# 10XGenomics/thermite

Measured on AMD Instinct MI355X. Metric: aligned reads/sec (91 bp), higher is better.
Workload: dtype i32

## Files before the change

thermite_amd/csrc/kernels_compact.hip:

```cpp
#include <hip/hip_runtime.h>

#include <algorithm>
#include <cstddef>
#include <cstdlib>

#include "launch.h"

namespace thm {
namespace dev {

constexpr uint32_t COMPACT_HEAVY_N = 8, COMPACT_CHUNK = 4;

struct CandRegs {
  uint32_t lo, hi;
};
static_assert(sizeof(Cand) == 112 && sizeof(thm_aln) == 112, "compact_emit permutes the dwords of these layouts");
static_assert(offsetof(Cand, ops_off) == 48 && offsetof(Cand, tx_ops_off) == 56 && offsetof(Cand, score) == 64 &&
                  offsetof(Cand, ops_len) == 80 && offsetof(Cand, tx_ops_len) == 84 && offsetof(Cand, strand) == 108 &&
                  offsetof(thm_aln, ops_off) == 24 && offsetof(thm_aln, tx_ops_off) == 56 && offsetof(thm_aln, xlen) == 80 &&
                  offsetof(thm_aln, ops_len) == 84 && offsetof(thm_aln, tx_ops_len) == 104 && offsetof(thm_aln, strand) == 108,
              "compact_emit permutes the dwords of these layouts");

__device__ __forceinline__ CandRegs cand_load(const Cand* c, int sub) {
  const uint32_t* w = reinterpret_cast<const uint32_t*>(c);
  CandRegs r;
  r.lo = w[sub];
  r.hi = sub < 12 ? w[16 + sub] : 0u;
  return r;
}

__device__ __forceinline__ uint32_t compact_emit(const CompactParams& p, const CandRegs c, uint64_t ai, uint64_t o, uint32_t xlen, bool primary, int sub) {
  const uint64_t ops_off = (uint64_t)__shfl(c.lo, 12, 16) | ((uint64_t)__shfl(c.lo, 13, 16) << 32);
  const uint64_t tx_ops_off = (uint64_t)__shfl(c.lo, 14, 16) | ((uint64_t)__shfl(c.lo, 15, 16) << 32);
  const uint32_t ops_len = __shfl(c.hi, 4, 16), tx_ops_len = __shfl(c.hi, 5, 16), flags = __shfl(c.hi, 11, 16);
  if (ai >= p.alns_cap || o + ops_len + tx_ops_len > p.ops_cap) return ops_len + tx_ops_len;
  auto copy_ops = [&](const uint8_t* src, uint8_t* dst, uint32_t len) {
    #pragma unroll 1
    for (uint32_t b0 = 0; b0 < len; b0 += 64) {
      uint8_t v[4];
      #pragma unroll
      for (int k = 0; k < 4; k++) {
        const uint32_t b = b0 + (uint32_t)sub + 16u * (uint32_t)k;
        v[k] = (b < len) ? src[b] : (uint8_t)0;
      }
      #pragma unroll
      for (int k = 0; k < 4; k++) {
        const uint32_t b = b0 + (uint32_t)sub + 16u * (uint32_t)k;
        if (b < len) dst[b] = v[k];
      }
    }
  };
  copy_ops(p.cand_ops + ops_off, p.ops + o, ops_len);
  const uint64_t go = o, to = o + ops_len;
  copy_ops(p.cand_ops + tx_ops_off, p.ops + to, tx_ops_len);
  const int src_lo = (int)((0x00BA987600543210ull >> (4 * sub)) & 15u);
  const int src_hi = (int)((0x0000B59876403210ull >> (4 * sub)) & 15u);
  uint32_t w0 = __shfl(c.lo, src_lo, 16), w1 = __shfl(c.hi, src_hi, 16);
  const uint64_t txo = ((flags >> 8) & 0xFFu) == THM_ALN_EXONIC ? to : 0ull;
  if (sub == 6) w0 = (uint32_t)go;
  if (sub == 7) w0 = (uint32_t)(go >> 32);
  if (sub == 14) w0 = (uint32_t)txo;
  if (sub == 15) w0 = (uint32_t)(txo >> 32);
  if (sub == 4) w1 = xlen;
  if (sub == 11) w1 = (flags & 0xFFu) | ((primary ? 1u : 0u) << 8) | (((flags >> 8) & 0xFFu) << 16);
  uint32_t* out = reinterpret_cast<uint32_t*>(p.alns + ai);
  out[sub] = w0;
  if (sub < 12) out[16 + sub] = w1;
  return ops_len + tx_ops_len;
}

__device__ __forceinline__ bool compact_faulted(const CompactParams& p) { return p.fault[0] != 0 || (p.fault[1] & FAULT_OPS_POOL) != 0; }

template <int K>
__global__ __launch_bounds__(256) void compact_kernel(CompactParams p) {
  const int sub = (int)(threadIdx.x & 15u);
  if (compact_faulted(p)) return;
  const uint64_t n_groups = (uint64_t)gridDim.x * 16, g = ((uint64_t)blockIdx.x * 256 + threadIdx.x) >> 4;
  for (uint64_t rb = g; rb < p.n_reads; rb += (uint64_t)K * n_groups) {
    uint32_t n[K], xlen[K], l0[K];
    uint64_t cand0[K], a0[K], o[K];
    #pragma unroll
    for (int k = 0; k < K; k++) {
      const uint64_t r = rb + (uint64_t)k * n_groups;
      n[k] = r < p.n_reads ? p.read_n_alns[r] : 0u;
    }
    #pragma unroll
    for (int k = 0; k < K; k++) {
      const uint64_t r = rb + (uint64_t)k * n_groups;
      if (n[k] > COMPACT_HEAVY_N) {
        if (sub == 0) {
          const unsigned long long h = atomicAdd(&p.heavy_cnt[0], 1ull);
          if (h < p.heavy_cap) p.heavy_list[h] = r;
        }
        n[k] = 0;
      }
      if (n[k]) {
        cand0[k] = p.read_cand_off[r];
        a0[k] = p.read_aln_off[r];
        o[k] = p.read_ops_off[r];
        xlen[k] = (uint32_t)(p.read_offsets[r + 1] - p.read_offsets[r]);
      }
    }
    #pragma unroll
    for (int k = 0; k < K; k++)
      if (n[k]) l0[k] = p.order[2 * cand0[k]];
    CandRegs cd[K];
    #pragma unroll
    for (int k = 0; k < K; k++)
      if (n[k]) cd[k] = cand_load(p.cands + cand0[k] + l0[k], sub);
    #pragma unroll
    for (int k = 0; k < K; k++) {
      if (!n[k]) continue;
      uint64_t ok = o[k] + compact_emit(p, cd[k], a0[k], o[k], xlen[k], true, sub);
      const uint32_t* la = p.order + 2 * cand0[k];
      for (uint32_t t = 1; t < n[k]; t++)
        ok += compact_emit(p, cand_load(p.cands + cand0[k] + la[t], sub), a0[k] + t, ok, xlen[k], false, sub);
    }
  }
}

__global__ __launch_bounds__(256) void compact_heavy_scan_kernel(CompactParams p) {
  __shared__ uint32_t wave_sum[4];
  __shared__ unsigned long long desc_base;
  if (compact_faulted(p)) return;
  const uint64_t H = min((unsigned long long)p.heavy_cap, p.heavy_cnt[0]);
  const int tid = (int)threadIdx.x, lane = tid & 63, wv = tid >> 6;
  for (uint64_t h = blockIdx.x; h < H; h += gridDim.x) {
    const uint64_t r = p.heavy_list[h];
    const uint32_t n = p.read_n_alns[r];
    const uint64_t cand0 = p.read_cand_off[r], a0 = p.read_aln_off[r];
    const Cand* cands = p.cands + cand0;
    const uint32_t* la = p.order + 2 * cand0;
    uint32_t carry = 0;
    for (uint32_t tile = 0; tile < n; tile += 256) {
      const uint32_t t = tile + (uint32_t)tid;
      uint32_t len = 0;
      if (t < n) {
        const Cand* cd = &cands[la[t]];
        len = cd->ops_len + cd->tx_ops_len;
      }
      uint32_t inc = len;
      #pragma unroll
      for (int o = 1; o < 64; o <<= 1) {
        const uint32_t v = __shfl_up(inc, o);
        if (lane >= o) inc += v;
      }
      if (lane == 63) wave_sum[wv] = inc;
      __syncthreads();
      uint32_t before = carry, total = 0;
      #pragma unroll
      for (int k = 0; k < 4; k++) {
        if (k < wv) before += wave_sum[k];
        total += wave_sum[k];
      }
      if (t < n && a0 + t < p.alns_cap) p.rel[a0 + t] = before + inc - len;
      carry += total;
      __syncthreads();
    }
    const uint32_t nd = (n + COMPACT_CHUNK - 1) / COMPACT_CHUNK;
    if (tid == 0) desc_base = atomicAdd(&p.heavy_cnt[1], (unsigned long long)nd);
    __syncthreads();
    const unsigned long long base = desc_base;
    for (uint32_t k = (uint32_t)tid; k < nd; k += 256)
      if (base + k < p.heavy_cap) p.heavy_desc[base + k] = (r << 24) | (uint64_t)k;
    __syncthreads();
  }
}

__global__ __launch_bounds__(256) void compact_heavy_copy_kernel(CompactParams p) {
  const int sub = (int)(threadIdx.x & 15u);
  if (compact_faulted(p)) return;
  const uint64_t D = min((unsigned long long)p.heavy_cap, p.heavy_cnt[1]);
  const uint64_t n_groups = (uint64_t)gridDim.x * 16;
  for (uint64_t d = ((uint64_t)blockIdx.x * 256 + threadIdx.x) >> 4; d < D; d += n_groups) {
    const uint64_t desc = p.heavy_desc[d], r = desc >> 24;
    const uint32_t t0 = (uint32_t)(desc & 0xFFFFFFu) * COMPACT_CHUNK, n = p.read_n_alns[r];
    const uint64_t cand0 = p.read_cand_off[r], a0 = p.read_aln_off[r], o0 = p.read_ops_off[r];
    const Cand* cands = p.cands + cand0;
    const uint32_t* la = p.order + 2 * cand0;
    const uint32_t xlen = (uint32_t)(p.read_offsets[r + 1] - p.read_offsets[r]);
    for (uint32_t t = t0; t < n && t < t0 + COMPACT_CHUNK; t++) {
      if (a0 + t >= p.alns_cap) break;
      (void)compact_emit(p, cand_load(&cands[la[t]], sub), a0 + t, o0 + p.rel[a0 + t], xlen, t == 0, sub);
    }
  }
}

}

int compact_k() {
  static const int v = [] {
    const char* e = getenv("THM_COMPACT_K");
    const int v = e ? atoi(e) : 2;
    return v == 1 || v == 2 || v == 4 ? v : 2;
  }();
  return v;
}

hipError_t launch_compact(const CompactParams& p, hipStream_t s) {
  static const unsigned n_cu = [] {
    int dev = 0, cu = 256;
    if (hipGetDevice(&dev) == hipSuccess) (void)hipDeviceGetAttribute(&cu, hipDeviceAttributeMultiprocessorCount, dev);
    return (unsigned)cu;
  }();
  const unsigned blocks = (unsigned)std::min<uint64_t>((p.n_reads + 15) / 16, (uint64_t)n_cu * 8);
  if (blocks == 0) return hipSuccess;
  const int k_reads = compact_k();
  if (k_reads == 1)
    hipLaunchKernelGGL(dev::compact_kernel<1>, dim3(blocks), dim3(256), 0, s, p);
  else if (k_reads == 2)
    hipLaunchKernelGGL(dev::compact_kernel<2>, dim3(blocks), dim3(256), 0, s, p);
  else
    hipLaunchKernelGGL(dev::compact_kernel<4>, dim3(blocks), dim3(256), 0, s, p);
  hipLaunchKernelGGL(dev::compact_heavy_scan_kernel, dim3(n_cu), dim3(256), 0, s, p);
  hipLaunchKernelGGL(dev::compact_heavy_copy_kernel, dim3(n_cu * 4), dim3(256), 0, s, p);
  return hipGetLastError();
}

}
```

Measured before the change: 93.87 million.

## Restructure compact kernel: per-alignment LDS work slots and dword-aligned ops copy

The compact kernel now gives each thread one read. Those threads stage per-alignment copy descriptors into shared-memory slots, and 16-lane groups then process alignments (not reads) in batches of K, issuing all loads before any stores. The byte-at-a-time ops copy is replaced by a dword copy aligned to the destination, with funnel shifts for source misalignment and single-byte head and tail handling, and a waitcnt separates the load and store phases. This aims to cut memory instructions and to balance work across lanes when reads carry different numbers of alignments. In exchange it adds shared-memory pressure, block-level syncs, serial descriptor generation per thread, and possible unaligned 32-bit source reads.

```diff
diff --git a/thermite_amd/csrc/compact_copy.h b/thermite_amd/csrc/compact_copy.h
--- /dev/null
+++ b/thermite_amd/csrc/compact_copy.h
@@ -0,0 +1,85 @@
+#ifndef THERMITE_COMPACT_COPY_H
+#define THERMITE_COMPACT_COPY_H
+#include <cstdint>
+
+#if defined(__HIPCC__)
+#define CCOPY_HD __host__ __device__ inline
+#else
+#define CCOPY_HD inline
+#endif
+
+namespace thm {
+namespace ccopy {
+
+constexpr int LANES = 16;
+constexpr int DWORDS_PER_LANE = 4;
+constexpr uint32_t TRIP_DWORDS = (uint32_t)(LANES * DWORDS_PER_LANE);
+constexpr uint32_t NO_BYTE = 0xFFFFFFFFu;
+constexpr int TAIL_LANE0 = 8;
+
+CCOPY_HD uint32_t head_bytes(uint64_t dst, uint32_t len) {
+  const uint32_t h = (uint32_t)(0 - dst) & 3u;
+  return h < len ? h : len;
+}
+CCOPY_HD uint32_t body_dwords(uint64_t dst, uint32_t len) { return (len - head_bytes(dst, len)) >> 2; }
+CCOPY_HD uint32_t tail_bytes(uint64_t dst, uint32_t len) { return (len - head_bytes(dst, len)) & 3u; }
+CCOPY_HD uint32_t trips(uint64_t dst, uint32_t len) {
+  const uint32_t nd = body_dwords(dst, len);
+  return nd ? (nd + TRIP_DWORDS - 1) / TRIP_DWORDS : (len ? 1u : 0u);
+}
+CCOPY_HD uint32_t lane_dword(int lane, int m, uint32_t trip) { return trip * TRIP_DWORDS + (uint32_t)m * LANES + (uint32_t)lane; }
+CCOPY_HD uint32_t edge_byte(int lane, uint64_t dst, uint32_t len) {
+  const uint32_t head = head_bytes(dst, len), tail = tail_bytes(dst, len);
+  if ((uint32_t)lane < head) return (uint32_t)lane;
+  if (lane >= TAIL_LANE0 && (uint32_t)(lane - TAIL_LANE0) < tail) return len - tail + (uint32_t)(lane - TAIL_LANE0);
+  return NO_BYTE;
+}
+CCOPY_HD uint32_t funnel(uint32_t lo, uint32_t hi, uint32_t shift) { return shift ? (lo >> (8 * shift)) | (hi << (32 - 8 * shift)) : lo; }
+
+struct LaneRegs {
+  uint32_t lo[DWORDS_PER_LANE], hi[DWORDS_PER_LANE];
+  uint32_t edge;
+};
+
+template <class M>
+CCOPY_HD void lane_load(const M& mem, uint64_t src, uint64_t dst, uint32_t len, uint32_t trip, int lane, LaneRegs& r) {
+  const uint32_t head = head_bytes(dst, len), nd = body_dwords(dst, len);
+#if defined(__HIPCC__)
+  #pragma unroll
+#endif
+  for (int m = 0; m < DWORDS_PER_LANE; m++) {
+    const uint32_t j = lane_dword(lane, m, trip);
+    r.lo[m] = r.hi[m] = 0u;
+    if (j < nd) {
+      const uint64_t s = src + head + 4ull * j;
+      r.lo[m] = mem.ld32(s & ~3ull);
+      if (s & 3u) r.hi[m] = mem.ld32((s & ~3ull) + 4);
+    }
+  }
+  r.edge = 0u;
+  if (trip == 0) {
+    const uint32_t e = edge_byte(lane, dst, len);
+    if (e != NO_BYTE) r.edge = mem.ld8(src + e);
+  }
+}
+
+template <class M>
+CCOPY_HD void lane_store(M& mem, uint64_t src, uint64_t dst, uint32_t len, uint32_t trip, int lane, const LaneRegs& r) {
+  const uint32_t head = head_bytes(dst, len), nd = body_dwords(dst, len);
+  const uint32_t shift = (uint32_t)(src + head) & 3u;
+#if defined(__HIPCC__)
+  #pragma unroll
+#endif
+  for (int m = 0; m < DWORDS_PER_LANE; m++) {
+    const uint32_t j = lane_dword(lane, m, trip);
+    if (j < nd) mem.st32(dst + head + 4ull * j, funnel(r.lo[m], r.hi[m], shift));
+  }
+  if (trip == 0) {
+    const uint32_t e = edge_byte(lane, dst, len);
+    if (e != NO_BYTE) mem.st8(dst + e, (uint8_t)r.edge);
+  }
+}
+
+}
+}
+#endif
diff --git a/thermite_amd/csrc/kernels_compact.hip b/thermite_amd/csrc/kernels_compact.hip
--- a/thermite_amd/csrc/kernels_compact.hip
+++ b/thermite_amd/csrc/kernels_compact.hip
@@ -4,6 +4,7 @@
 #include <cstddef>
 #include <cstdlib>
 
+#include "compact_copy.h"
 #include "launch.h"
 
 namespace thm {
@@ -14,12 +15,12 @@
 struct CandRegs {
   uint32_t lo, hi;
 };
-static_assert(sizeof(Cand) == 112 && sizeof(thm_aln) == 112, "compact_emit permutes the dwords of these layouts");
+static_assert(sizeof(Cand) == 112 && sizeof(thm_aln) == 112, "emit_record permutes the dwords of these layouts");
 static_assert(offsetof(Cand, ops_off) == 48 && offsetof(Cand, tx_ops_off) == 56 && offsetof(Cand, score) == 64 &&
                   offsetof(Cand, ops_len) == 80 && offsetof(Cand, tx_ops_len) == 84 && offsetof(Cand, strand) == 108 &&
                   offsetof(thm_aln, ops_off) == 24 && offsetof(thm_aln, tx_ops_off) == 56 && offsetof(thm_aln, xlen) == 80 &&
                   offsetof(thm_aln, ops_len) == 84 && offsetof(thm_aln, tx_ops_len) == 104 && offsetof(thm_aln, strand) == 108,
-              "compact_emit permutes the dwords of these layouts");
+              "emit_record permutes the dwords of these layouts");
 
 __device__ __forceinline__ CandRegs cand_load(const Cand* c, int sub) {
   const uint32_t* w = reinterpret_cast<const uint32_t*>(c);
@@ -29,93 +30,139 @@
   return r;
 }
 
-__device__ __forceinline__ uint32_t compact_emit(const CompactParams& p, const CandRegs c, uint64_t ai, uint64_t o, uint32_t xlen, bool primary, int sub) {
-  const uint64_t ops_off = (uint64_t)__shfl(c.lo, 12, 16) | ((uint64_t)__shfl(c.lo, 13, 16) << 32);
-  const uint64_t tx_ops_off = (uint64_t)__shfl(c.lo, 14, 16) | ((uint64_t)__shfl(c.lo, 15, 16) << 32);
-  const uint32_t ops_len = __shfl(c.hi, 4, 16), tx_ops_len = __shfl(c.hi, 5, 16), flags = __shfl(c.hi, 11, 16);
-  if (ai >= p.alns_cap || o + ops_len + tx_ops_len > p.ops_cap) return ops_len + tx_ops_len;
-  auto copy_ops = [&](const uint8_t* src, uint8_t* dst, uint32_t len) {
+struct OpsMem {
+  const uint8_t* src;
+  uint8_t* dst;
+  __device__ __forceinline__ uint32_t ld32(uint64_t o) const { return *reinterpret_cast<const uint32_t*>(src + o); }
+  __device__ __forceinline__ uint32_t ld8(uint64_t o) const { return src[o]; }
+  __device__ __forceinline__ void st32(uint64_t o, uint32_t v) { *reinterpret_cast<uint32_t*>(dst + o) = v; }
+  __device__ __forceinline__ void st8(uint64_t o, uint8_t v) { dst[o] = v; }
+};
+
+struct AlnCopy {
+  CandRegs c;
+  ccopy::LaneRegs gx, tx;
+  uint64_t gx_src, tx_src, o;
+  uint32_t gx_len, tx_len;
+
+  __device__ __forceinline__ void load(const CompactParams& p, const Cand* cand, uint64_t gx_src_, uint64_t tx_src_, uint32_t gx_len_, uint32_t tx_len_,
+                                       uint64_t o_, int sub) {
+    gx_src = gx_src_, tx_src = tx_src_, gx_len = gx_len_, tx_len = tx_len_, o = o_;
+    const OpsMem mem{p.cand_ops, p.ops};
+    c = cand_load(cand, sub);
+    ccopy::lane_load(mem, gx_src, o, gx_len, 0, sub, gx);
+    ccopy::lane_load(mem, tx_src, o + gx_len, tx_len, 0, sub, tx);
+  }
+
+  static __device__ __forceinline__ void loads_done() { __builtin_amdgcn_s_waitcnt(0x0F70); }
+
+  __device__ __forceinline__ void store(const CompactParams& p, uint64_t ai, uint32_t xlen, bool primary, int sub) {
+    OpsMem mem{p.cand_ops, p.ops};
+    const uint64_t go = o, to = o + gx_len;
+    ccopy::lane_store(mem, gx_src, go, gx_len, 0, sub, gx);
+    ccopy::lane_store(mem, tx_src, to, tx_len, 0, sub, tx);
     #pragma unroll 1
-    for (uint32_t b0 = 0; b0 < len; b0 += 64) {
-      uint8_t v[4];
-      #pragma unroll
-      for (int k = 0; k < 4; k++) {
-        const uint32_t b = b0 + (uint32_t)sub + 16u * (uint32_t)k;
-        v[k] = (b < len) ? src[b] : (uint8_t)0;
-      }
-      #pragma unroll
-      for (int k = 0; k < 4; k++) {
-        const uint32_t b = b0 + (uint32_t)sub + 16u * (uint32_t)k;
-        if (b < len) dst[b] = v[k];
-      }
-    }
-  };
-  copy_ops(p.cand_ops + ops_off, p.ops + o, ops_len);
-  const uint64_t go = o, to = o + ops_len;
-  copy_ops(p.cand_ops + tx_ops_off, p.ops + to, tx_ops_len);
-  const int src_lo = (int)((0x00BA987600543210ull >> (4 * sub)) & 15u);
-  const int src_hi = (int)((0x0000B59876403210ull >> (4 * sub)) & 15u);
-  uint32_t w0 = __shfl(c.lo, src_lo, 16), w1 = __shfl(c.hi, src_hi, 16);
-  const uint64_t txo = ((flags >> 8) & 0xFFu) == THM_ALN_EXONIC ? to : 0ull;
-  if (sub == 6) w0 = (uint32_t)go;
-  if (sub == 7) w0 = (uint32_t)(go >> 32);
-  if (sub == 14) w0 = (uint32_t)txo;
-  if (sub == 15) w0 = (uint32_t)(txo >> 32);
-  if (sub == 4) w1 = xlen;
-  if (sub == 11) w1 = (flags & 0xFFu) | ((primary ? 1u : 0u) << 8) | (((flags >> 8) & 0xFFu) << 16);
-  uint32_t* out = reinterpret_cast<uint32_t*>(p.alns + ai);
-  out[sub] = w0;
-  if (sub < 12) out[16 + sub] = w1;
-  return ops_len + tx_ops_len;
-}
+    for (uint32_t trip = 1; trip < ccopy::trips(go, gx_len); trip++) {
+      ccopy::lane_load(mem, gx_src, go, gx_len, trip, sub, gx);
+      loads_done();
+      ccopy::lane_store(mem, gx_src, go, gx_len, trip, sub, gx);
+    }
+    #pragma unroll 1
+    for (uint32_t trip = 1; trip < ccopy::trips(to, tx_len); trip++) {
+      ccopy::lane_load(mem, tx_src, to, tx_len, trip, sub, tx);
+      loads_done();
+      ccopy::lane_store(mem, tx_src, to, tx_len, trip, sub, tx);
+    }
+    const uint32_t flags = __shfl(c.hi, 11, 16);
+    const int src_lo = (int)((0x00BA987600543210ull >> (4 * sub)) & 15u);
+    const int src_hi = (int)((0x0000B59876403210ull >> (4 * sub)) & 15u);
+    uint32_t w0 = __shfl(c.lo, src_lo, 16), w1 = __shfl(c.hi, src_hi, 16);
+    const uint64_t txo = ((flags >> 8) & 0xFFu) == THM_ALN_EXONIC ? to : 0ull;
+    if (sub == 6) w0 = (uint32_t)go;
+    if (sub == 7) w0 = (uint32_t)(go >> 32);
+    if (sub == 14) w0 = (uint32_t)txo;
+    if (sub == 15) w0 = (uint32_t)(txo >> 32);
+    if (sub == 4) w1 = xlen;
+    if (sub == 11) w1 = (flags & 0xFFu) | ((primary ? 1u : 0u) << 8) | (((flags >> 8) & 0xFFu) << 16);
+    uint32_t* out = reinterpret_cast<uint32_t*>(p.alns + ai);
+    out[sub] = w0;
+    if (sub < 12) out[16 + sub] = w1;
+  }
+};
 
 __device__ __forceinline__ bool compact_faulted(const CompactParams& p) { return p.fault[0] != 0 || (p.fault[1] & FAULT_OPS_POOL) != 0; }
 
+constexpr uint32_t COMPACT_TILE = 256, COMPACT_SLOTS = 512;
+constexpr uint64_t NO_CAND = ~0ull;
+
 template <int K>
-__global__ __launch_bounds__(256) void compact_kernel(CompactParams p) {
-  const int sub = (int)(threadIdx.x & 15u);
+__global__ __launch_bounds__(COMPACT_TILE) void compact_kernel(CompactParams p) {
+  __shared__ uint64_t s_cand[COMPACT_SLOTS], s_gx[COMPACT_SLOTS], s_tx[COMPACT_SLOTS], s_o[COMPACT_SLOTS];
+  __shared__ uint32_t s_gx_len[COMPACT_SLOTS], s_tx_len[COMPACT_SLOTS], s_xlen[COMPACT_SLOTS];
+  __shared__ uint8_t s_primary[COMPACT_SLOTS];
   if (compact_faulted(p)) return;
-  const uint64_t n_groups = (uint64_t)gridDim.x * 16, g = ((uint64_t)blockIdx.x * 256 + threadIdx.x) >> 4;
-  for (uint64_t rb = g; rb < p.n_reads; rb += (uint64_t)K * n_groups) {
-    uint32_t n[K], xlen[K], l0[K];
-    uint64_t cand0[K], a0[K], o[K];
-    #pragma unroll
-    for (int k = 0; k < K; k++) {
-      const uint64_t r = rb + (uint64_t)k * n_groups;
-      n[k] = r < p.n_reads ? p.read_n_alns[r] : 0u;
-    }
-    #pragma unroll
-    for (int k = 0; k < K; k++) {
-      const uint64_t r = rb + (uint64_t)k * n_groups;
-      if (n[k] > COMPACT_HEAVY_N) {
-        if (sub == 0) {
-          const unsigned long long h = atomicAdd(&p.heavy_cnt[0], 1ull);
-          if (h < p.heavy_cap) p.heavy_list[h] = r;
-        }
-        n[k] = 0;
-      }
-      if (n[k]) {
-        cand0[k] = p.read_cand_off[r];
-        a0[k] = p.read_aln_off[r];
-        o[k] = p.read_ops_off[r];
-        xlen[k] = (uint32_t)(p.read_offsets[r + 1] - p.read_offsets[r]);
-      }
-    }
-    #pragma unroll
-    for (int k = 0; k < K; k++)
-      if (n[k]) l0[k] = p.order[2 * cand0[k]];
-    CandRegs cd[K];
-    #pragma unroll
-    for (int k = 0; k < K; k++)
-      if (n[k]) cd[k] = cand_load(p.cands + cand0[k] + l0[k], sub);
-    #pragma unroll
-    for (int k = 0; k < K; k++) {
-      if (!n[k]) continue;
-      uint64_t ok = o[k] + compact_emit(p, cd[k], a0[k], o[k], xlen[k], true, sub);
-      const uint32_t* la = p.order + 2 * cand0[k];
-      for (uint32_t t = 1; t < n[k]; t++)
-        ok += compact_emit(p, cand_load(p.cands + cand0[k] + la[t], sub), a0[k] + t, ok, xlen[k], false, sub);
-    }
+  const uint32_t tid = threadIdx.x;
+  const int sub = (int)(tid & 15u);
+  const uint32_t grp = tid >> 4;
+  const uint64_t r0 = (uint64_t)blockIdx.x * COMPACT_TILE, r = r0 + tid;
+  const uint64_t r_end = min((unsigned long long)(r0 + COMPACT_TILE), (unsigned long long)p.n_reads);
+  const uint64_t aln_base = p.read_aln_off[r0], n_slots = p.read_aln_off[r_end] - aln_base;
+  uint32_t n = 0, xlen = 0;
+  uint64_t cand0 = 0, a0 = 0, o = 0;
+  if (r < p.n_reads) {
+    n = p.read_n_alns[r];
+    cand0 = p.read_cand_off[r];
+    a0 = p.read_aln_off[r];
+    o = p.read_ops_off[r];
+    xlen = (uint32_t)(p.read_offsets[r + 1] - p.read_offsets[r]);
+  }
+  if (n > COMPACT_HEAVY_N) {
+    const unsigned long long h = atomicAdd(&p.heavy_cnt[0], 1ull);
+    if (h < p.heavy_cap) p.heavy_list[h] = r;
+    n = 0;
+  }
+  uint32_t t = 0;
+  for (uint64_t c0 = 0; c0 < n_slots; c0 += COMPACT_SLOTS) {
+    const uint32_t cnt = (uint32_t)min((unsigned long long)COMPACT_SLOTS, (unsigned long long)(n_slots - c0));
+    for (uint32_t i = tid; i < cnt; i += COMPACT_TILE) s_cand[i] = NO_CAND;
+    __syncthreads();
+    while (t < n && a0 + t - aln_base < c0 + COMPACT_SLOTS) {
+      const uint32_t slot = (uint32_t)(a0 + t - aln_base - c0);
+      const uint64_t ci = cand0 + p.order[2 * cand0 + t];
+      const Cand* cd = p.cands + ci;
+      const uint64_t gx_src = cd->ops_off, tx_src = cd->tx_ops_off;
+      const uint32_t gx_len = cd->ops_len, tx_len = cd->tx_ops_len;
+      if (a0 + t < p.alns_cap && o + gx_len + tx_len <= p.ops_cap) {
+        s_cand[slot] = ci;
+        s_gx[slot] = gx_src;
+        s_tx[slot] = tx_src;
+        s_o[slot] = o;
+        s_gx_len[slot] = gx_len;
+        s_tx_len[slot] = tx_len;
+        s_xlen[slot] = xlen;
+        s_primary[slot] = t == 0;
+      }
+      o += gx_len + tx_len;
+      t++;
+    }
+    __syncthreads();
+    for (uint32_t b = 0; b < cnt; b += 16 * K) {
+      AlnCopy ac[K];
+      bool live[K];
+      #pragma unroll
+      for (int k = 0; k < K; k++) {
+        const uint32_t d = b + grp + 16u * (uint32_t)k;
+        live[k] = d < cnt && s_cand[d] != NO_CAND;
+        if (live[k]) ac[k].load(p, p.cands + s_cand[d], s_gx[d], s_tx[d], s_gx_len[d], s_tx_len[d], s_o[d], sub);
+      }
+      AlnCopy::loads_done();
+      #pragma unroll
+      for (int k = 0; k < K; k++) {
+        const uint32_t d = b + grp + 16u * (uint32_t)k;
+        if (live[k]) ac[k].store(p, aln_base + c0 + d, s_xlen[d], s_primary[d] != 0, sub);
+      }
+    }
+    __syncthreads();
   }
 }
 
@@ -181,7 +228,14 @@
     const uint32_t xlen = (uint32_t)(p.read_offsets[r + 1] - p.read_offsets[r]);
     for (uint32_t t = t0; t < n && t < t0 + COMPACT_CHUNK; t++) {
       if (a0 + t >= p.alns_cap) break;
-      (void)compact_emit(p, cand_load(&cands[la[t]], sub), a0 + t, o0 + p.rel[a0 + t], xlen, t == 0, sub);
+      const Cand* cd = &cands[la[t]];
+      const uint32_t gx_len = cd->ops_len, tx_len = cd->tx_ops_len;
+      const uint64_t o = o0 + p.rel[a0 + t];
+      if (o + gx_len + tx_len > p.ops_cap) continue;
+      AlnCopy ac;
+      ac.load(p, cd, cd->ops_off, cd->tx_ops_off, gx_len, tx_len, o, sub);
+      AlnCopy::loads_done();
+      ac.store(p, a0 + t, xlen, t == 0, sub);
     }
   }
 }
@@ -203,15 +257,15 @@
     if (hipGetDevice(&dev) == hipSuccess) (void)hipDeviceGetAttribute(&cu, hipDeviceAttributeMultiprocessorCount, dev);
     return (unsigned)cu;
   }();
-  const unsigned blocks = (unsigned)std::min<uint64_t>((p.n_reads + 15) / 16, (uint64_t)n_cu * 8);
+  const unsigned blocks = (unsigned)((p.n_reads + dev::COMPACT_TILE - 1) / dev::COMPACT_TILE);
   if (blocks == 0) return hipSuccess;
-  const int k_reads = compact_k();
-  if (k_reads == 1)
-    hipLaunchKernelGGL(dev::compact_kernel<1>, dim3(blocks), dim3(256), 0, s, p);
-  else if (k_reads == 2)
-    hipLaunchKernelGGL(dev::compact_kernel<2>, dim3(blocks), dim3(256), 0, s, p);
+  const int k_alns = compact_k();
+  if (k_alns == 1)
+    hipLaunchKernelGGL(dev::compact_kernel<1>, dim3(blocks), dim3(dev::COMPACT_TILE), 0, s, p);
+  else if (k_alns == 2)
+    hipLaunchKernelGGL(dev::compact_kernel<2>, dim3(blocks), dim3(dev::COMPACT_TILE), 0, s, p);
   else
-    hipLaunchKernelGGL(dev::compact_kernel<4>, dim3(blocks), dim3(256), 0, s, p);
+    hipLaunchKernelGGL(dev::compact_kernel<4>, dim3(blocks), dim3(dev::COMPACT_TILE), 0, s, p);
   hipLaunchKernelGGL(dev::compact_heavy_scan_kernel, dim3(n_cu), dim3(256), 0, s, p);
   hipLaunchKernelGGL(dev::compact_heavy_copy_kernel, dim3(n_cu * 4), dim3(256), 0, s, p);
   return hipGetLastError();
```

Result: faster. 96.03 million, median of 6 (+2.3%).
